# cdcseacave/openMVS

Measured on AMD Instinct MI355X. Metric: Mpix/s depth-map output at 1920x1080 N-view, higher is better.
Workload: dtype f32

## Files before the change

### openmvs_amd/csrc/pm_band.hip

```cpp
#pragma once

#ifndef PM_NDRAW
#define PM_NDRAW 6
#endif
#ifndef PM_BAND_MINWAVES
#define PM_BAND_MINWAVES 3
#endif
#ifndef PM_BAND_MINWAVES_PHOTO
#define PM_BAND_MINWAVES_PHOTO 4
#endif
#ifndef PM_BAND_MINWAVES_PHOTO
#define PM_BAND_MINWAVES_PHOTO 4
#endif

struct PMPix {
	float depth, nx, ny, nz, conf;
	float p0, p1, scaleRange, depthRange;
	int st, it, idxScale, flags;
	float hd, hnx, hny, hnz, hp0, hp1;
	int hst, pad0;
	float nb[2][5];
	float qX[4][3], qn[4][3];
	float vx, vy, normSq0, sumW;
	double X0x, X0y;
	int x, y;
	float x1[2];
	double hr[3];
	float dr[PM_NDRAW][3];
};
#if defined(__HIP_DEVICE_COMPILE__)
#define PM_LDS __attribute__((address_space(3)))
template <class T> __device__ __forceinline__ PM_LDS T* pm_launder(T* p) { PM_LDS T* q = (PM_LDS T*)p; asm volatile("" : "+v"(q)); return q; }
#else
#define PM_LDS
template <class T> __device__ __forceinline__ T* pm_launder(T* p) { return p; }
#endif
enum { PMF_SMOOTH = 1, PMF_CHANGED = 2, PMF_POK0 = 4, PMF_POK1 = 8 };

template <int G, int VPL, bool GEO, bool BUF, bool TILED>
__device__ __forceinline__ void pm_visit(const PMTask& t, const PMKParams& kp, const PMImgBuf& rs, uint32_t pass, int sgn, float2* s_wg, PMPix* s_pixg, const double* hotBase,
		int g, int v, int slot, bool active, int x, int y, int ySafe, size_t idx, const bool* bok, const int* qxs, const int* qys, const size_t* qis, unsigned oldMask,
		float n0D, float n0N0, float n0N1, float n0N2, float n0C, float n1D, float n1N0, float n1N1, float n1N2, float n1C,
		float& rD, float& rN0, float& rN1, float& rN2, float& rC, bool& wr PM_PROF_ARG) {
	constexpr int NBD = PM_SRC_HOT + (GEO ? PM_SRC_GEO : 0);
	const pm_gf gDepth = pm_globw(t.depth), gNormal = pm_globw(t.normal), gConf = pm_globw(t.conf);
	const int yTop = ySafe;
	float oDepth = 0.f, oNx = 0.f, oNy = 0.f, oNz = 0.f, oConf = 2.f, prior = 0.f;
	float myD = 0.f, myN0 = 0.f, myN1 = 0.f, myN2 = 1.f;
	unsigned char maskByte = 1;
	if (active) {
		if (t.prior) prior = pm_glob(t.prior)[idx];
		if (t.mask != nullptr) maskByte = t.mask[idx];
		if (slot == 0) { myD = bok[0] ? n0D : 0.f; myN0 = n0N0; myN1 = n0N1; myN2 = n0N2; }
		else if (slot == 1) { myD = bok[1] ? n1D : 0.f; myN0 = n1N0; myN1 = n1N1; myN2 = n1N2; }
		else {
			const size_t qi = slot == 2 ? qis[2] : qis[3];
			const bool old = TILED && ((oldMask >> slot) & 1u);
			const pm_gcf sD = pm_glob(old ? t.depthOld : t.depth), sN = pm_glob(old ? t.normalOld : t.normal);
			myD = sD[qi]; myN0 = sN[qi * 3]; myN1 = sN[qi * 3 + 1]; myN2 = sN[qi * 3 + 2];
		}
		oDepth = gDepth[idx]; oNx = gNormal[idx * 3]; oNy = gNormal[idx * 3 + 1]; oNz = gNormal[idx * 3 + 2]; oConf = gConf[idx];
	}
	float normSq0, sumW;
	pm_fill_patch<G, true>(t, active, active ? x : PM_HW, active ? y : yTop, v, s_wg, normSq0, sumW);
	const bool masked = active && maskByte == 0;
	const bool valid = active && !masked && !(normSq0 < kp.thMagnitudeSq && !(prior > 0));
	if (v == 0) s_wg[PM_NT] = make_float2(prior, prior > 0 ? pm_expf(normSq0 * (-1.f / (1.f * 0.02f))) : 0.f);
	{
		PM_LDS PMPix* P = pm_launder(s_pixg);
		const bool bk = slot == 0 ? bok[0] : slot == 1 ? bok[1] : slot == 2 ? bok[2] : bok[3];
		const bool okS = valid && bk && myD > 0;
		const unsigned long long bal = __ballot(okS);
		const unsigned closeMask = (unsigned)((bal >> (g * G)) & 0xFull);
		if (v < 4) {
			const int qx = slot == 0 ? qxs[0] : slot == 1 ? qxs[1] : slot == 2 ? qxs[2] : qxs[3];
			const int qy = slot == 0 ? qys[0] : slot == 1 ? qys[1] : slot == 2 ? qys[2] : qys[3];
			const double z = (double)myD;
			P->qX[slot][0] = okS ? (float)(((double)qx - t.cx) * z / t.fx) : 0.f;
			P->qX[slot][1] = okS ? (float)(((double)qy - t.cy) * z / t.fy) : 0.f;
			P->qX[slot][2] = okS ? (float)z : 0.f;
			P->qn[slot][0] = okS ? myN0 : 0.f; P->qn[slot][1] = okS ? myN1 : 0.f; P->qn[slot][2] = okS ? myN2 : 1.f;
		}
		if (v == 0) {
			const double X0x = ((double)x - t.cx) / t.fx, X0y = ((double)y - t.cy) / t.fy;
			P->X0x = X0x; P->X0y = X0y; P->vx = (float)X0x; P->vy = (float)X0y; P->normSq0 = normSq0; P->sumW = sumW; P->x = x; P->y = y;
			P->depth = valid ? oDepth : 0.f; P->nx = valid ? oNx : 0.f; P->ny = valid ? oNy : 0.f; P->nz = valid ? oNz : 0.f; P->conf = valid ? oConf : 2.f;
			P->p0 = 0.f; P->p1 = 0.f; P->scaleRange = 1.f; P->depthRange = 0.f;
			enum { ST_PROP0 = 0, ST_DONE = 5 };
			P->st = valid ? ST_PROP0 : ST_DONE; P->it = 0; P->idxScale = 0;
			P->flags = PMF_SMOOTH | ((closeMask & 1u) ? PMF_POK0 : 0) | ((closeMask & 2u) ? PMF_POK1 : 0) | (int)(closeMask << 8);
			P->nb[0][0] = n0D; P->nb[0][1] = n0N0; P->nb[0][2] = n0N1; P->nb[0][3] = n0N2; P->nb[0][4] = n0C;
			P->nb[1][0] = n1D; P->nb[1][1] = n1N0; P->nb[1][2] = n1N1; P->nb[1][3] = n1N2; P->nb[1][4] = n1C;
		}
		if (v < 2)
			P->x1[v] = v == 0 ? (float)(((double)(x + sgn) - t.cx) / t.fx) : (float)(((double)(y + sgn) - t.cy) / t.fy);
		const unsigned nd = min((unsigned)PM_NDRAW, kp.nRandomIters);
		for (unsigned it0 = 0; it0 < nd; it0 += G) {
			const unsigned itv = it0 + (unsigned)v;
			const PmPhilox4 r = pm_philox4x32_10((uint32_t)x, (uint32_t)y, (uint32_t)(PM_STREAM_REFINE * 256) + itv, 0u, t.k0, t.k1base + pass);
			if (itv < (unsigned)PM_NDRAW) {
				P->dr[itv][0] = 2.f * pm_u32_to_unit(r.v[0]) - 1.f; P->dr[itv][1] = 2.f * pm_u32_to_unit(r.v[1]) - 1.f; P->dr[itv][2] = 2.f * pm_u32_to_unit(r.v[2]) - 1.f;
			}
		}
	}
	__syncthreads();
	PM_TICK(12); PM_COUNT(9, 1);
	enum { ST_PROP0 = 0, ST_PROP1 = 1, ST_DECIDE = 2, ST_RAND = 3, ST_REFINE = 4, ST_DONE = 5 };
	const uint32_t k1 = t.k1base + pass;
	for (;;) {
		bool need = false;
		float hd = 0.f, hnx = 0.f, hny = 0.f, hnz = 1.f;
		{
			PM_LDS PMPix* P = pm_launder(s_pixg);
			int st = P->st; unsigned it = (unsigned)P->it, idxScale = (unsigned)P->idxScale; int flags = P->flags;
			const int px = P->x, py = P->y;
			const float vx = P->vx, vy = P->vy, vz = 1.f;
			float scaleRange = P->scaleRange, depthRange = P->depthRange, p0 = P->p0, p1 = P->p1;
			float hp0 = 0.f, hp1 = 0.f; int hst = ST_DONE;
			while (!need && st != ST_DONE) {
				if (st <= ST_PROP1) {
					const bool vert = (st == ST_PROP1); ++st;
					const bool pok = (flags & (vert ? PMF_POK1 : PMF_POK0)) != 0;
					const PM_LDS float* nbp = P->nb[vert ? 1 : 0];
					const float cd = nbp[0], cnx = nbp[1], cny = nbp[2], cnz = nbp[3], pconf = nbp[4];
					hd = cd; hnx = cnx; hny = cny; hnz = cnz;
					if (pok && pconf < kp.thKeep) {
						float depthNew = cd; bool zero;
						{
							const float nx1 = vert ? vy : vx, cn = vert ? cny : cnx;
							const float denom = cnz + nx1 * cn;
							zero = pm_fabsf(denom) < 0.0001f;
							const float x1 = P->x1[vert ? 1 : 0];
							const float nom = cd * (cnz + x1 * cn);
							if (!zero) depthNew = nom / denom;
						}
						hd = (!zero && pm_in_range(depthNew, t.dMin, t.dMax)) ? depthNew : cd;
						hnx = cnx; hny = cny; hnz = cnz;
						pm_correct_normal(vx, vy, vz, hnx, hny, hnz);
						need = true; hst = ST_PROP0;
					}
				} else if (st == ST_DECIDE) {
					const float conf = P->conf;
					if (conf <= kp.thConfSmall) idxScale = 2;
					else if (conf <= kp.thConfBig) idxScale = 1;
					else if (conf >= kp.thConfRand) { flags &= ~PMF_SMOOTH; st = ST_RAND; it = 0; continue; }
					scaleRange = pm_pow2neg(idxScale);
					depthRange = P->depth * kp.depthRatio;
					p0 = pm_atan2f(P->ny, P->nx); p1 = pm_acosf(pm_clampf(P->nz, -1.f, 1.f));
					st = ST_REFINE; it = 0;
				} else if (st == ST_RAND) {
					if (it >= kp.nRandomIters) { st = ST_DONE; break; }
					const PmPhilox4 r = pm_philox4x32_10((uint32_t)px, (uint32_t)py, (uint32_t)(PM_STREAM_RAND * 256) + it, 0u, t.k0, k1);
					++it;
					const float rr = t.dMinSqr + (t.dMaxSqr - t.dMinSqr) * pm_u32_to_unit(r.v[0]);
					hd = rr * rr;
					pm_random_normal(pm_u32_to_unit(r.v[1]), pm_u32_to_unit(r.v[2]), vx, vy, vz, hnx, hny, hnz);
					need = true; hst = ST_RAND;
				} else {
					if (it >= kp.nRandomIters) { st = ST_DONE; break; }
					float e0, e1, e2;
					if (it < (unsigned)PM_NDRAW) { e0 = P->dr[it][0]; e1 = P->dr[it][1]; e2 = P->dr[it][2]; }
					else {
						const PmPhilox4 r = pm_philox4x32_10((uint32_t)px, (uint32_t)py, (uint32_t)(PM_STREAM_REFINE * 256) + it, 0u, t.k0, k1);
						e0 = 2.f * pm_u32_to_unit(r.v[0]) - 1.f; e1 = 2.f * pm_u32_to_unit(r.v[1]) - 1.f; e2 = 2.f * pm_u32_to_unit(r.v[2]) - 1.f;
					}
					++it;
					const float ndepth = P->depth + (depthRange * scaleRange) * e0;
					if (!pm_in_range(ndepth, t.dMin, t.dMax)) continue;
					hp0 = p0 + (kp.angle1Range * scaleRange) * e1;
					hp1 = p1 + (kp.angle2Range * scaleRange) * e2;
					pm_dir2normal_quad(hp0, hp1, v, hnx, hny, hnz);
					if (hnx * vx + hny * vy + hnz * vz >= 0) continue;
					hd = ndepth;
					need = true; hst = ST_REFINE;
				}
			}
			double hr0 = 0.0, hr1 = 0.0, hr2 = 0.0;
			if (need) pm_homography_plane(P->X0x, P->X0y, hd, hnx, hny, hnz, hr0, hr1, hr2);
			__builtin_amdgcn_wave_barrier();
			if (v == 0) {
				P->hr[0] = hr0; P->hr[1] = hr1; P->hr[2] = hr2;
				P->st = st; P->it = (int)it; P->idxScale = (int)idxScale; P->flags = flags;
				P->scaleRange = scaleRange; P->depthRange = depthRange; P->p0 = p0; P->p1 = p1;
				P->hd = hd; P->hnx = hnx; P->hny = hny; P->hnz = hnz; P->hp0 = hp0; P->hp1 = hp1; P->hst = hst;
			}
		}
		const unsigned long long needBal = __ballot(need);
		if (needBal == 0ull) break;
		PM_TICK(1); PM_COUNT(8, __popcll(needBal)); PM_HIST(__popcll(needBal) / G);
		float sf0, sf1, sf2, sf3;
		{
			const PM_LDS PMPix* P = pm_launder(s_pixg);
			const int flags = P->flags;
			const bool on = need && (flags & PMF_SMOOTH) && ((flags >> (8 + slot)) & 1);
			float myF = 1.f;
			if (on) {
				const float vx = P->vx, vy = P->vy;
				const float q0 = P->qX[slot][0], q1 = P->qX[slot][1], q2 = P->qX[slot][2], m0 = P->qn[slot][0], m1 = P->qn[slot][1], m2 = P->qn[slot][2];
				const float planeD = -hd * (hnx * vx + hny * vy + hnz * 1.f);
				const float dist = (hnx * q0 + (hny * q1 + hnz * q2)) + planeD;
				const float r = dist / hd;
				const float factorDepth = pm_expf((r * r) * kp.smoothSigmaDepth);
				const float ca = pm_clampf((hnx * m0 + hny * m1 + hnz * m2) / pm_sqrtf((hnx * hnx + hny * hny + hnz * hnz) * (m0 * m0 + m1 * m1 + m2 * m2)), -1.f, 1.f);
				const float ac = pm_acosf(ca);
				const float factorNormal = pm_expf((ac * ac) * kp.smoothSigmaNormal);
				myF = (1.f - kp.smoothBonusDepth * factorDepth) * (1.f - kp.smoothBonusNormal * factorNormal);
			}
			sf0 = pm_quad_bcast<0>(myF); sf1 = pm_quad_bcast<1>(myF); sf2 = pm_quad_bcast<2>(myF); sf3 = pm_quad_bcast<3>(myF);
		}
		PM_TICK(2);
		float sc = PM_INF, sc2 = PM_INF;
		{
			const PM_LDS PMPix* P = pm_launder(s_pixg);
#pragma unroll 1
			for (int u = 0; u < VPL; ++u) {
				const int vw = v + u * G;
				if (need && vw < t.nSrc) {
					const float s1 = pm_score_view<GEO, BUF ? 2 : 1, true, true>(t.src[vw], t, kp, P->x, P->y, P->X0x, P->X0y, P->normSq0, P->sumW, s_wg, hd, hnx, hny, hnz, sf0, sf1, sf2, sf3, 0.f,
						hotBase + vw * NBD, hotBase + vw * NBD + PM_SRC_HOT, rs PM_PROF_PASS, (const double*)P->hr);
					if (s1 < sc) { sc2 = sc; sc = s1; } else if (s1 < sc2) sc2 = s1;
				}
			}
		}
		const float nconf = pm_aggregate<G>(sc, t.nSrc, kp.thRobust, sc2);
		{
			PM_LDS PMPix* P = pm_launder(s_pixg);
			if (need && v == 0 && P->conf > nconf) {
				P->conf = nconf; P->depth = P->hd; P->nx = P->hnx; P->ny = P->hny; P->nz = P->hnz;
				int flags = P->flags | PMF_CHANGED;
				P->flags = flags;
				const int hst = P->hst;
				if (hst == ST_RAND) { if (nconf < kp.thConfRand) P->st = ST_DECIDE; }
				else if (hst == ST_REFINE) { P->p0 = P->hp0; P->p1 = P->hp1; const int is = P->idxScale + 1; P->idxScale = is; P->scaleRange = pm_pow2neg((unsigned)is); }
			}
		}
		__builtin_amdgcn_wave_barrier();
		PM_TICK(6);
	}
	{
		const PM_LDS PMPix* P = pm_launder(s_pixg);
		wr = (P->flags & PMF_CHANGED) && valid;
		rD = wr ? P->depth : oDepth; rN0 = wr ? P->nx : oNx; rN1 = wr ? P->ny : oNy; rN2 = wr ? P->nz : oNz; rC = wr ? P->conf : oConf;
	}
}

template <int G, int VPL, bool GEO, bool BUF, bool TILED>
__global__ __launch_bounds__(64, (GEO ? PM_BAND_MINWAVES : PM_BAND_MINWAVES_PHOTO)) void pm_sweep2_kernel(const PMTask* __restrict__ tasks, PMKParams kp, PMStep st, uint32_t pass) {
	constexpr int PPW = 64 / G;
	constexpr int NV = G * VPL;
	constexpr int NBD = PM_SRC_HOT + (GEO ? PM_SRC_GEO : 0);
	static_assert(G >= 4, "a pixel gets at least a quad of lanes");
	PM_PROF_DECL;
	__shared__ float2 s_w[PPW][PM_NT + 1];
	__shared__ double s_src[NV * NBD];
	__shared__ PMPix s_pix[PPW];
	unsigned vbx = blockIdx.x, vby = blockIdx.y;
	{
		const unsigned nbx = gridDim.x, nwg = nbx * gridDim.y, orig = blockIdx.y * nbx + blockIdx.x;
		const unsigned xcd = orig % 8u, q = nwg / 8u, r = nwg % 8u;
		const unsigned wgid = (xcd < r ? xcd * (q + 1u) : r * (q + 1u) + (xcd - r) * q) + orig / 8u;
		vby = wgid / nbx; vbx = wgid - vby * nbx;
	}
	const PMTask& t = tasks[vby];
	const PMImgBuf rs = pm_make_imgbuf(t);
	const int lane = threadIdx.x;
	for (int i = lane; i < NV * NBD; i += 64) s_src[i] = ((const double*)&t.src[i / NBD])[i % NBD];
	const int g = lane / G, v = lane % G, slot = v & 3;
	const int w = t.w, h = t.h;
	const PMStepPix sp = pm_step_pixel<TILED>(st, w, h, (int)vbx * PPW + g);
	const bool active = sp.active;
	const int x = sp.x, y = sp.y;
	const size_t idx = (size_t)y * w + x;
	const int sgn = st.dir == 0 ? -1 : 1;
	bool bok[4]; int qxs[4], qys[4]; size_t qis[4];
#pragma unroll
	for (int k = 0; k < 4; ++k) {
		const int ox = (k == 0) ? sgn : (k == 2 ? -sgn : 0), oy = (k == 1) ? sgn : (k == 3 ? -sgn : 0);
		bool ok;
		if (ox == -1) ok = x > PM_HW; else if (ox == 1) ok = x < w - PM_HW; else if (oy == -1) ok = y > PM_HW; else ok = y < h - PM_HW;
		bok[k] = ok && active; qxs[k] = x + ox; qys[k] = y + oy;
		qis[k] = bok[k] ? (size_t)(y + oy) * w + (x + ox) : idx;
	}
	const pm_gf gDepth = pm_globw(t.depth), gNormal = pm_globw(t.normal), gConf = pm_globw(t.conf);
	float n0D = 0.f, n0N0 = 0.f, n0N1 = 0.f, n0N2 = 0.f, n0C = 2.f, n1D = 0.f, n1N0 = 0.f, n1N1 = 0.f, n1N2 = 0.f, n1C = 2.f;
	if (active) {
		const size_t q0 = qis[0], q1 = qis[1];
		if (TILED) {
			const pm_gcf nD0 = pm_glob((sp.oldMask & 1u) ? t.depthOld : t.depth), nN0 = pm_glob((sp.oldMask & 1u) ? t.normalOld : t.normal), nC0 = pm_glob((sp.oldMask & 1u) ? t.confOld : t.conf);
			const pm_gcf nD1 = pm_glob((sp.oldMask & 2u) ? t.depthOld : t.depth), nN1 = pm_glob((sp.oldMask & 2u) ? t.normalOld : t.normal), nC1 = pm_glob((sp.oldMask & 2u) ? t.confOld : t.conf);
			n0D = nD0[q0]; n0N0 = nN0[q0 * 3]; n0N1 = nN0[q0 * 3 + 1]; n0N2 = nN0[q0 * 3 + 2]; n0C = nC0[q0];
			n1D = nD1[q1]; n1N0 = nN1[q1 * 3]; n1N1 = nN1[q1 * 3 + 1]; n1N2 = nN1[q1 * 3 + 2]; n1C = nC1[q1];
		} else {
			n0D = gDepth[q0]; n0N0 = gNormal[q0 * 3]; n0N1 = gNormal[q0 * 3 + 1]; n0N2 = gNormal[q0 * 3 + 2]; n0C = gConf[q0];
			n1D = gDepth[q1]; n1N0 = gNormal[q1 * 3]; n1N1 = gNormal[q1 * 3 + 1]; n1N2 = gNormal[q1 * 3 + 2]; n1C = gConf[q1];
		}
	}
	__syncthreads();
	float rD, rN0, rN1, rN2, rC; bool wr;
	pm_visit<G, VPL, GEO, BUF, TILED>(t, kp, rs, pass, sgn, s_w[g], &s_pix[g], s_src, g, v, slot, active, x, y, active ? y : PM_HW, active ? idx : (size_t)PM_HW * w + PM_HW, bok, qxs, qys, qis, sp.oldMask,
		n0D, n0N0, n0N1, n0N2, n0C, n1D, n1N0, n1N1, n1N2, n1C, rD, rN0, rN1, rN2, rC, wr PM_PROF_PASS);
	if (wr && v == 0) { gDepth[idx] = rD; gNormal[idx * 3] = rN0; gNormal[idx * 3 + 1] = rN1; gNormal[idx * 3 + 2] = rN2; gConf[idx] = rC; }
	PM_PROF_FLUSH();
}
```

### openmvs_amd/csrc/pm_kernels.hip

```cpp
#pragma once
#include <hip/hip_runtime.h>
#include <cstddef>
#include "pm_math.h"

#define PM_MAX_SRC 16
#ifndef PM_BLOCK
#define PM_BLOCK 64
#endif
typedef const float __attribute__((address_space(1)))* pm_gcf;
typedef float __attribute__((address_space(1)))* pm_gf;
#if defined(__HIP_DEVICE_COMPILE__)
typedef float pm_f4v __attribute__((ext_vector_type(4)));
typedef const pm_f4v __attribute__((address_space(1)))* pm_gcf4;
__device__ __forceinline__ pm_gcf4 pm_glob4(const float4* p) { return (pm_gcf4)p; }
__device__ __forceinline__ pm_f4v pm_loadq(pm_gcf4 base, unsigned off) { return base[off]; }
#else
typedef const float4* pm_gcf4;
__device__ __forceinline__ pm_gcf4 pm_glob4(const float4* p) { return p; }
__device__ __forceinline__ float4 pm_loadq(pm_gcf4 base, unsigned off) { return base[off]; }
#endif
__device__ __forceinline__ pm_gcf pm_glob(const float* p) { return (pm_gcf)p; }
__device__ __forceinline__ pm_gf pm_globw(float* p) { return (pm_gf)p; }
#define PM_HW 4
#define PM_NT 25
// ... 132 lines not shown
#pragma unroll
				for (int k = 0; k < 3; ++k) t += O[i * 3 + k] * O[k * 3 + j];
				Rm[i * 3 + j] = ((i == j ? 1.f : 0.f) + O[i * 3 + j] * s) + t * (1.f - c);
			}
		const float r0 = Rm[0] * nx + Rm[1] * ny + Rm[2] * nz;
		const float r1 = Rm[3] * nx + Rm[4] * ny + Rm[5] * nz;
		const float r2 = Rm[6] * nx + Rm[7] * ny + Rm[8] * nz;
		nx = r0; ny = r1; nz = r2;
	}
}

#define PM_DPP_F(v, ctrl) __int_as_float(__builtin_amdgcn_update_dpp(__float_as_int(v), __float_as_int(v), (ctrl), 0xf, 0xf, false))
template <int G>
__device__ __forceinline__ void pm_group_min2(float s, float s2, float& m1, float& m2) {
	float a = s, b = s2;
#define PM_MIN2_STEP(ctrl) { const float oa = PM_DPP_F(a, ctrl), ob = PM_DPP_F(b, ctrl); \
		const float na = pm_minf(a, oa), nb = pm_minf(pm_maxf(a, oa), pm_minf(b, ob)); a = na; b = nb; }
	if (G >= 2) PM_MIN2_STEP(0xB1)
	if (G >= 4) PM_MIN2_STEP(0x4E)
	if (G >= 8) PM_MIN2_STEP(0x141)
	if (G >= 16) PM_MIN2_STEP(0x140)
#undef PM_MIN2_STEP
	m1 = a; m2 = b;
}
template <int K> __device__ __forceinline__ float pm_quad_bcast(float v) { return PM_DPP_F(v, K * 0x55); }

__device__ __forceinline__ void pm_dir2normal_quad(float p0, float p1, int v, float& nx, float& ny, float& nz) {
	float s, c;
	pm_sincosf((v & 1) ? p1 : p0, &s, &c);
	const float sx = pm_quad_bcast<0>(s), cx = pm_quad_bcast<0>(c), sy = pm_quad_bcast<1>(s), cy = pm_quad_bcast<1>(c);
	nx = cx * sy; ny = sx * sy; nz = cy;
}

__device__ __forceinline__ void pm_homography_plane(double X0x, double X0y, float depth, float nx, float ny, float nz, double& r0, double& r1, double& r2) {
	const double n0 = (double)nx, n1 = (double)ny, n2 = (double)nz;
	const double ndx = (n0 * X0x + n1 * X0y) + n2;
	const double den = ndx * (double)depth;
	const double inv = (den == 0.0) ? 1e+14 : 1.0 / den;
	r0 = n0 * inv; r1 = n1 * inv; r2 = n2 * inv;
}
__device__ __forceinline__ void pm_homography(const double* hlm, const PMTask& t, double X0x, double X0y,
		float depth, float nx, float ny, float nz, float* H, const double* rpre = nullptr) {
	double Hl[9], Hm[3];
#pragma unroll
	for (int i = 0; i < 9; ++i) Hl[i] = hlm[i];
#pragma unroll
	for (int i = 0; i < 3; ++i) Hm[i] = hlm[9 + i];
	double r0, r1, r2;
	if (rpre) { r0 = rpre[0]; r1 = rpre[1]; r2 = rpre[2]; }
	else pm_homography_plane(X0x, X0y, depth, nx, ny, nz, r0, r1, r2);
#pragma unroll
	for (int i = 0; i < 3; ++i) {
		const double hm = Hm[i];
		const double m0 = Hl[i * 3 + 0] + hm * r0;
		const double m1 = Hl[i * 3 + 1] + hm * r1;
		const double m2 = Hl[i * 3 + 2] + hm * r2;
		if (t.hrUpper) {
			H[i * 3 + 0] = (float)(m0 * t.Hr[0]);
			H[i * 3 + 1] = (float)(m1 * t.Hr[4]);
			H[i * 3 + 2] = (float)((m0 * t.Hr[2] + m1 * t.Hr[5]) + m2 * t.Hr[8]);
		} else {
#pragma unroll
			for (int j = 0; j < 3; ++j)
				H[i * 3 + j] = (float)((m0 * t.Hr[j] + m1 * t.Hr[3 + j]) + m2 * t.Hr[6 + j]);
		}
	}
}

#ifndef PM_WIDE_MINWAVES
#define PM_WIDE_MINWAVES 3
#endif

#if defined(__HIP_DEVICE_COMPILE__)
typedef int pm_rsrc __attribute__((ext_vector_type(4)));
__device__ __forceinline__ pm_rsrc pm_make_rsrc(const void* base, unsigned count, unsigned stride = 16) {
	const unsigned long long b = (unsigned long long)base;
	pm_rsrc r;
	r.x = __builtin_amdgcn_readfirstlane((int)(unsigned)b);
	r.y = __builtin_amdgcn_readfirstlane((int)(((unsigned)(b >> 32) & 0xffffu) | (stride << 16)));
	r.z = __builtin_amdgcn_readfirstlane((int)count);
	r.w = 0x00020000;
	return r;
}
__device__ __forceinline__ void pm_bufload5(pm_f4v& q0, pm_f4v& q1, pm_f4v& q2, pm_f4v& q3, pm_f4v& q4, unsigned i0, unsigned i1, unsigned i2, unsigned i3, unsigned i4, pm_rsrc r) {
	asm volatile("buffer_load_dwordx4 %0, %5, %10, 0 idxen\n\tbuffer_load_dwordx4 %1, %6, %10, 0 idxen\n\tbuffer_load_dwordx4 %2, %7, %10, 0 idxen\n\t"
	             "buffer_load_dwordx4 %3, %8, %10, 0 idxen\n\tbuffer_load_dwordx4 %4, %9, %10, 0 idxen"
		: "=&v"(q0), "=&v"(q1), "=&v"(q2), "=&v"(q3), "=&v"(q4) : "v"(i0), "v"(i1), "v"(i2), "v"(i3), "v"(i4), "s"(r) : "memory");
}
template <int LEFT>
__device__ __forceinline__ void pm_bufwait5(pm_f4v& q0, pm_f4v& q1, pm_f4v& q2, pm_f4v& q3, pm_f4v& q4) {
	asm volatile("s_waitcnt vmcnt(%5)" : "+v"(q0), "+v"(q1), "+v"(q2), "+v"(q3), "+v"(q4) : "i"(LEFT));
}
__device__ __forceinline__ unsigned pm_mad24(int a, int b, unsigned c) { unsigned r; asm("v_mad_u32_u24 %0, %1, %2, %3" : "=v"(r) : "v"(a), "v"(b), "v"(c)); return r; }
#else
typedef float4 pm_f4v;
struct pm_rsrc { const float4* base; unsigned count; };
__device__ __forceinline__ pm_rsrc pm_make_rsrc(const void* base, unsigned count) { return pm_rsrc{(const float4*)base, count}; }
__device__ __forceinline__ void pm_bufload5(pm_f4v& q0, pm_f4v& q1, pm_f4v& q2, pm_f4v& q3, pm_f4v& q4, unsigned i0, unsigned i1, unsigned i2, unsigned i3, unsigned i4, pm_rsrc r) {
	const float4 z = make_float4(0.f, 0.f, 0.f, 0.f);
	q0 = i0 < r.count ? r.base[i0] : z; q1 = i1 < r.count ? r.base[i1] : z; q2 = i2 < r.count ? r.base[i2] : z; q3 = i3 < r.count ? r.base[i3] : z; q4 = i4 < r.count ? r.base[i4] : z;
}
template <int LEFT> __device__ __forceinline__ void pm_bufwait5(pm_f4v&, pm_f4v&, pm_f4v&, pm_f4v&, pm_f4v&) {}
__device__ __forceinline__ unsigned pm_mad24(int a, int b, unsigned c) { return (unsigned)(((unsigned)a & 0xffffffu) * ((unsigned)b & 0xffffffu)) + c; }
#endif

struct PMImgBuf { pm_rsrc rs; };
__device__ __forceinline__ PMImgBuf pm_make_imgbuf(const PMTask& t) {
	PMImgBuf b;
	b.rs = pm_make_rsrc(t.qArr, t.qCount);
	return b;
}

template <bool QUAD>
__device__ __forceinline__ void pm_tap_row_global(const pm_gcf img, int sw, int sh, float h0, float h3, float h6, float X0, float X1, float X2,
		const float2* wrow, float& sum, float& sumSq, float& num, bool& oob)
{
	const int lxMax = sw - 2, lyMax = sh - 2;
	float fxs[5], fys[5];
	unsigned offs[5];
#pragma unroll
	for (int j = 0; j < 5; ++j) {
		float ptx, pty;
		pm_div2(X0, X1, X2, &ptx, &pty);
		oob = oob || !pm_inside1(ptx, pty, sw, sh);
		int lx = (int)ptx, ly = (int)pty;
		fxs[j] = ptx - (float)lx; fys[j] = pty - (float)ly;
		lx = min(max(lx, 0), lxMax); ly = min(max(ly, 0), lyMax);
		offs[j] = QUAD ? 4u * ((unsigned)(lx + ly) * (unsigned)sh + (unsigned)ly) : (unsigned)ly * (unsigned)sw + (unsigned)lx;
		X0 += h0; X1 += h3; X2 += h6;
	}
	float v00[5], v01[5], v10[5], v11[5];
#pragma unroll
	for (int j = 0; j < 5; ++j) {
		const pm_gcf p = img + offs[j];
		if (QUAD) { v00[j] = p[0]; v01[j] = p[1]; v10[j] = p[2]; v11[j] = p[3]; }
		else { v00[j] = p[0]; v01[j] = p[1]; v10[j] = p[sw]; v11[j] = p[sw + 1]; }
	}
#pragma unroll
// ... 51 lines not shown
		sumSq += v * vw;
		num += v * pw.y;
	}
}
template <bool BUF>
__device__ __forceinline__ void pm_taps_fast(const PMImgBuf& rs, unsigned qbase, const pm_gcf4 imgQ, int sw, int sh, const float* H, float bX0, float bX1, float bX2,
		const float2* wts, float& sum, float& sumSq, float& num, PMTapRange& rg)
{
	PMRowPos pa, pb; PMRowQ qa, qb;
	pm_row_issue<BUF, true>(rs, qbase, imgQ, sw, sh, H[0], H[3], H[6], bX0, bX1, bX2, pa, qa, rg);
#pragma unroll 1
	for (int i = 0; i < 4; i += 2) {
		bX0 += H[1]; bX1 += H[4]; bX2 += H[7];
		pm_row_issue<BUF, false>(rs, qbase, imgQ, sw, sh, H[0], H[3], H[6], bX0, bX1, bX2, pb, qb, rg);
		PM_SCHED_BARRIER();
		pm_row_consume<BUF, 5>(pa, qa, wts + i * 5, sum, sumSq, num);
		PM_SCHED_BARRIER();
		bX0 += H[1]; bX1 += H[4]; bX2 += H[7];
		pm_row_issue<BUF, false>(rs, qbase, imgQ, sw, sh, H[0], H[3], H[6], bX0, bX1, bX2, pa, qa, rg);
		PM_SCHED_BARRIER();
		pm_row_consume<BUF, 5>(pb, qb, wts + (i + 1) * 5, sum, sumSq, num);
		PM_SCHED_BARRIER();
	}
	pm_range_corner(rg, pa.ptx[0], pa.pty[0], bX2);
	pm_range_corner(rg, pa.ptx[4], pa.pty[4], (((bX2 + H[6]) + H[6]) + H[6]) + H[6]);
	pm_row_consume<BUF, 0>(pa, qa, wts + 20, sum, sumSq, num);
}

template <bool GEO, int MODE, bool PF = false, bool EARLY = false>
__device__ __forceinline__ float pm_score_view(const PMSrcView& s, const PMTask& t, const PMKParams& kp,
		int x, int y, double X0x, double X0y, float normSq0, float sumW, const float2* wts,
		float depth, float nx, float ny, float nz,
		float sf0, float sf1, float sf2, float sf3, float prior,
		const double* hot, const double* geoTab, const PMImgBuf& rs PM_PROF_ARG, const double* rpre = nullptr)
{
	const int sw = ((const int*)(hot + 12))[0], sh = ((const int*)(hot + 12))[1];
	float H[9];
	pm_homography(hot, t, X0x, X0y, depth, nx, ny, nz, H, rpre);
	PM_TICK(3);
	const float px = (float)(x - PM_HW), py = (float)(y - PM_HW);
	const float X0 = H[0] * px + H[1] * py + H[2];
	const float X1 = H[3] * px + H[4] * py + H[5];
	const float X2 = H[6] * px + H[7] * py + H[8];
	float bX0 = X0, bX1 = X1, bX2 = X2;
#pragma unroll
	for (int i = 0; i < 9; ++i) H[i] *= 2.f;
	float sum = 0.f, sumSq = 0.f, num = 0.f;
	bool oob = false;
	if (MODE == 0) {
#pragma unroll 1
		for (int i = 0; i < 5; ++i) {
			pm_tap_row_global<false>(pm_glob(s.img), sw, sh, H[0], H[3], H[6], bX0, bX1, bX2, wts + i * 5, sum, sumSq, num, oob);
			bX0 += H[1]; bX1 += H[4]; bX2 += H[7];
		}
	} else {
		const bool sane = pm_fabsf(X0) + 8.f * (pm_fabsf(H[0]) + pm_fabsf(H[1])) < 5e17f && pm_fabsf(X1) + 8.f * (pm_fabsf(H[3]) + pm_fabsf(H[4])) < 5e17f
			&& pm_fabsf(X2) + 8.f * (pm_fabsf(H[6]) + pm_fabsf(H[7])) < 5e11f;
		if (EARLY && sane) {
			bool outside = false;
			float cx, cy;
			if (bX2 >= 9.094947e-13f && bX2 <= 1.0995116e12f) { pm_div2_inrange(bX0, bX1, bX2, &cx, &cy); outside = !pm_inside1(cx, cy, sw, sh); }
			float c0 = bX0, c1 = bX1, c2 = bX2;
#pragma unroll
			for (int i = 0; i < 4; ++i) { c0 += H[1]; c1 += H[4]; c2 += H[7]; }
#pragma unroll
			for (int j = 0; j < 4; ++j) { c0 += H[0]; c1 += H[3]; c2 += H[6]; }
			if (c2 >= 9.094947e-13f && c2 <= 1.0995116e12f) { pm_div2_inrange(c0, c1, c2, &cx, &cy); outside = outside || !pm_inside1(cx, cy, sw, sh); }
// ... 17 lines not shown
			oob = !cornersIn;
			if (cornersIn && !allIn) {
				float cX0 = rX0, cX1 = rX1, cX2 = rX2;
#pragma unroll 1
				for (int i = 0; i < 5; ++i) {
					float X0t = cX0, X1t = cX1, X2t = cX2;
#pragma unroll 1
					for (int j = 0; j < 5; ++j) {
						float ptx, pty;
						pm_div2_inrange(X0t, X1t, X2t, &ptx, &pty);
						oob = oob || !pm_inside1(ptx, pty, sw, sh);
						X0t += H[0]; X1t += H[3]; X2t += H[6];
					}
					cX0 += H[1]; cX1 += H[4]; cX2 += H[7];
				}
			}
		} else {
			sum = 0.f; sumSq = 0.f; num = 0.f;
			bX0 = rX0; bX1 = rX1; bX2 = rX2;
#pragma unroll 1
			for (int i = 0; i < 5; ++i) {
				pm_tap_row_global<true>(pm_glob((const float*)s.imgQ), sw, sh, H[0], H[3], H[6], bX0, bX1, bX2, wts + i * 5, sum, sumSq, num, oob);
				bX0 += H[1]; bX1 += H[4]; bX2 += H[7];
			}
		}
	}
	PM_TICK(4);
	if (oob) return kp.thRobust;
	const float normSq1 = sumSq - (sum * sum) / sumW;
	const float nrmSq = normSq0 * normSq1;
	if (nrmSq <= 1e-16f) return kp.thRobust;
	const float ncc = pm_clampf(num / pm_sqrtf(nrmSq), -1.f, 1.f);
	float score = 1.f - ncc;
	score *= sf0; score *= sf1; score *= sf2; score *= sf3;
	if (GEO) {
		const float* gt = (const float*)geoTab;
		const float* sdepth = *(const float* const*)(geoTab + 12);
		const int dw = ((const int*)(geoTab + 13))[0], dh = ((const int*)(geoTab + 13))[1];
		float Tl[9], Tm[3], Tr[9], Tn[3];
#pragma unroll
		for (int i = 0; i < 9; ++i) { Tl[i] = gt[i]; Tr[i] = gt[12 + i]; }
#pragma unroll
		for (int i = 0; i < 3; ++i) { Tm[i] = gt[9 + i]; Tn[i] = gt[21 + i]; }
#pragma unroll
		for (int i = 0; i < 9; ++i) PM_OPAQUE(Tr[i]);
#pragma unroll
		for (int i = 0; i < 3; ++i) PM_OPAQUE(Tn[i]);
		if (sdepth != nullptr) {
			float consistency = 4.f;
			const float Xc0 = (float)X0x * depth, Xc1 = (float)X0y * depth, Xc2 = depth;
			const float Y0 = (Tl[0] * Xc0 + Tl[1] * Xc1 + Tl[2] * Xc2) + Tm[0];
			const float Y1 = (Tl[3] * Xc0 + Tl[4] * Xc1 + Tl[5] * Xc2) + Tm[1];
			const float Y2 = (Tl[6] * Xc0 + Tl[7] * Xc1 + Tl[8] * Xc2) + Tm[2];
			if (Y2 > 0) {
				const float x1x = Y0 / Y2, x1y = Y1 / Y2;
				if (pm_inside1(x1x, x1y, dw, dh)) {
					const int lx = (int)x1x, ly = (int)x1y;
					const float fx = x1x - (float)lx, fx1 = 1.f - fx;
					const float fy = x1y - (float)ly, fy1 = 1.f - fy;
					const pm_gcf p = pm_glob(sdepth) + (size_t)ly * dw + lx;
					const float x0y0 = p[0], x1y0 = p[1], x0y1 = p[dw], x1y1 = p[dw + 1];
					const bool b00 = pm_fabsf(Y2 - x0y0) / Y2 < 0.03f, b10 = pm_fabsf(Y2 - x1y0) / Y2 < 0.03f;
					const bool b01 = pm_fabsf(Y2 - x0y1) / Y2 < 0.03f, b11 = pm_fabsf(Y2 - x1y1) / Y2 < 0.03f;
					if (b00 || b10 || b01 || b11) {
						const float depth1 =
							fy1 * (fx1 * (b00 ? x0y0 : (b10 ? x1y0 : (b01 ? x0y1 : x1y1))) + fx * (b10 ? x1y0 : (b00 ? x0y0 : (b11 ? x1y1 : x0y1)))) +
// ... 494 lines not shown
```

Baseline: 55.85.

## Switch band kernel lane mapping from pixel-major to view-major groups

Lanes are remapped so that consecutive lanes hold different pixels for the same view slot (g = lane % PPW, v = lane / PPW). Neighbouring pixels' texture gathers for one view then sit in the same quads, and per-pixel loads are restricted to the lanes that need them. Reductions and the normal construction move from quad DPP broadcasts to cross-lane xor shuffles at stride PPW, and smoothness factors go through LDS (nb is reused as scratch) instead of quad broadcasts. A host-side gather census instrumentation is added behind a compile flag. The risks are costlier cross-lane shuffles and extra LDS traffic with wave barriers.

```diff
diff --git a/openmvs_amd/csrc/pm_band.hip b/openmvs_amd/csrc/pm_band.hip
--- a/openmvs_amd/csrc/pm_band.hip
+++ b/openmvs_amd/csrc/pm_band.hip
@@ -13,13 +13,13 @@
 #define PM_BAND_MINWAVES_PHOTO 4
 #endif
 
-struct PMPix {
+struct alignas(16) PMPix {
+	float nb[2][5];
 	float depth, nx, ny, nz, conf;
 	float p0, p1, scaleRange, depthRange;
 	int st, it, idxScale, flags;
 	float hd, hnx, hny, hnz, hp0, hp1;
 	int hst, pad0;
-	float nb[2][5];
 	float qX[4][3], qn[4][3];
 	float vx, vy, normSq0, sumW;
 	double X0x, X0y;
@@ -35,43 +35,49 @@
 #define PM_LDS
 template <class T> __device__ __forceinline__ T* pm_launder(T* p) { return p; }
 #endif
+static_assert(sizeof(PMPix) == 368, "sixteen of them, the weights and the views' matrices fit a sixteenth of a CU's LDS (tests/test_kernel_resources.py)");
+__device__ __forceinline__ PM_LDS float* pm_pix_sf(PM_LDS PMPix* P) { return P->nb[0]; }
 enum { PMF_SMOOTH = 1, PMF_CHANGED = 2, PMF_POK0 = 4, PMF_POK1 = 8 };
 
 template <int G, int VPL, bool GEO, bool BUF, bool TILED>
 __device__ __forceinline__ void pm_visit(const PMTask& t, const PMKParams& kp, const PMImgBuf& rs, uint32_t pass, int sgn, float2* s_wg, PMPix* s_pixg, const double* hotBase,
-		int g, int v, int slot, bool active, int x, int y, int ySafe, size_t idx, const bool* bok, const int* qxs, const int* qys, const size_t* qis, unsigned oldMask,
+		int g, int v, bool active, int x, int y, int ySafe, size_t idx, const bool* bok, const int* qxs, const int* qys, const size_t* qis, unsigned oldMask,
 		float n0D, float n0N0, float n0N1, float n0N2, float n0C, float n1D, float n1N0, float n1N1, float n1N2, float n1C,
 		float& rD, float& rN0, float& rN1, float& rN2, float& rC, bool& wr PM_PROF_ARG) {
 	constexpr int NBD = PM_SRC_HOT + (GEO ? PM_SRC_GEO : 0);
+	constexpr int PPW = 64 / G;
+	const int slot = v & 3;
 	const pm_gf gDepth = pm_globw(t.depth), gNormal = pm_globw(t.normal), gConf = pm_globw(t.conf);
 	const int yTop = ySafe;
 	float oDepth = 0.f, oNx = 0.f, oNy = 0.f, oNz = 0.f, oConf = 2.f, prior = 0.f;
 	float myD = 0.f, myN0 = 0.f, myN1 = 0.f, myN2 = 1.f;
 	unsigned char maskByte = 1;
-	if (active) {
-		if (t.prior) prior = pm_glob(t.prior)[idx];
-		if (t.mask != nullptr) maskByte = t.mask[idx];
-		if (slot == 0) { myD = bok[0] ? n0D : 0.f; myN0 = n0N0; myN1 = n0N1; myN2 = n0N2; }
-		else if (slot == 1) { myD = bok[1] ? n1D : 0.f; myN0 = n1N0; myN1 = n1N1; myN2 = n1N2; }
+	if (active && v < 4) {
+		if (v == 0) {
+			if (t.prior) prior = pm_glob(t.prior)[idx];
+			if (t.mask != nullptr) maskByte = t.mask[idx];
+			oDepth = gDepth[idx]; oNx = gNormal[idx * 3]; oNy = gNormal[idx * 3 + 1]; oNz = gNormal[idx * 3 + 2]; oConf = gConf[idx];
+			myD = bok[0] ? n0D : 0.f; myN0 = n0N0; myN1 = n0N1; myN2 = n0N2;
+		}
+		else if (v == 1) { myD = bok[1] ? n1D : 0.f; myN0 = n1N0; myN1 = n1N1; myN2 = n1N2; }
 		else {
 			const size_t qi = slot == 2 ? qis[2] : qis[3];
 			const bool old = TILED && ((oldMask >> slot) & 1u);
 			const pm_gcf sD = pm_glob(old ? t.depthOld : t.depth), sN = pm_glob(old ? t.normalOld : t.normal);
 			myD = sD[qi]; myN0 = sN[qi * 3]; myN1 = sN[qi * 3 + 1]; myN2 = sN[qi * 3 + 2];
 		}
-		oDepth = gDepth[idx]; oNx = gNormal[idx * 3]; oNy = gNormal[idx * 3 + 1]; oNz = gNormal[idx * 3 + 2]; oConf = gConf[idx];
 	}
 	float normSq0, sumW;
 	pm_fill_patch<G, true>(t, active, active ? x : PM_HW, active ? y : yTop, v, s_wg, normSq0, sumW);
-	const bool masked = active && maskByte == 0;
-	const bool valid = active && !masked && !(normSq0 < kp.thMagnitudeSq && !(prior > 0));
+	const bool valid0 = v == 0 && active && maskByte != 0 && !(normSq0 < kp.thMagnitudeSq && !(prior > 0));
+	const bool valid = ((__ballot(valid0) >> g) & 1ull) != 0;
 	if (v == 0) s_wg[PM_NT] = make_float2(prior, prior > 0 ? pm_expf(normSq0 * (-1.f / (1.f * 0.02f))) : 0.f);
 	{
 		PM_LDS PMPix* P = pm_launder(s_pixg);
 		const bool bk = slot == 0 ? bok[0] : slot == 1 ? bok[1] : slot == 2 ? bok[2] : bok[3];
 		const bool okS = valid && bk && myD > 0;
-		const unsigned long long bal = __ballot(okS);
-		const unsigned closeMask = (unsigned)((bal >> (g * G)) & 0xFull);
+		const unsigned long long bal = __ballot(okS) >> g;
+		const unsigned closeMask = (unsigned)((bal & 1ull) | ((bal >> (PPW - 1)) & 2ull) | ((bal >> (2 * PPW - 2)) & 4ull) | ((bal >> (3 * PPW - 3)) & 8ull));
 		if (v < 4) {
 			const int qx = slot == 0 ? qxs[0] : slot == 1 ? qxs[1] : slot == 2 ? qxs[2] : qxs[3];
 			const int qy = slot == 0 ? qys[0] : slot == 1 ? qys[1] : slot == 2 ? qys[2] : qys[3];
@@ -89,11 +95,11 @@
 			enum { ST_PROP0 = 0, ST_DONE = 5 };
 			P->st = valid ? ST_PROP0 : ST_DONE; P->it = 0; P->idxScale = 0;
 			P->flags = PMF_SMOOTH | ((closeMask & 1u) ? PMF_POK0 : 0) | ((closeMask & 2u) ? PMF_POK1 : 0) | (int)(closeMask << 8);
-			P->nb[0][0] = n0D; P->nb[0][1] = n0N0; P->nb[0][2] = n0N1; P->nb[0][3] = n0N2; P->nb[0][4] = n0C;
-			P->nb[1][0] = n1D; P->nb[1][1] = n1N0; P->nb[1][2] = n1N1; P->nb[1][3] = n1N2; P->nb[1][4] = n1C;
-		}
-		if (v < 2)
+		}
+		if (v < 2) {
+			P->nb[v][0] = v == 0 ? n0D : n1D; P->nb[v][1] = v == 0 ? n0N0 : n1N0; P->nb[v][2] = v == 0 ? n0N1 : n1N1; P->nb[v][3] = v == 0 ? n0N2 : n1N2; P->nb[v][4] = v == 0 ? n0C : n1C;
 			P->x1[v] = v == 0 ? (float)(((double)(x + sgn) - t.cx) / t.fx) : (float)(((double)(y + sgn) - t.cy) / t.fy);
+		}
 		const unsigned nd = min((unsigned)PM_NDRAW, kp.nRandomIters);
 		for (unsigned it0 = 0; it0 < nd; it0 += G) {
 			const unsigned itv = it0 + (unsigned)v;
@@ -108,6 +114,7 @@
 	enum { ST_PROP0 = 0, ST_PROP1 = 1, ST_DECIDE = 2, ST_RAND = 3, ST_REFINE = 4, ST_DONE = 5 };
 	const uint32_t k1 = t.k1base + pass;
 	for (;;) {
+		PM_CENSUS_TRIP();
 		bool need = false;
 		float hd = 0.f, hnx = 0.f, hny = 0.f, hnz = 1.f;
 		{
@@ -169,7 +176,7 @@
 					if (!pm_in_range(ndepth, t.dMin, t.dMax)) continue;
 					hp0 = p0 + (kp.angle1Range * scaleRange) * e1;
 					hp1 = p1 + (kp.angle2Range * scaleRange) * e2;
-					pm_dir2normal_quad(hp0, hp1, v, hnx, hny, hnz);
+					pm_dir2normal_vm<PPW>(hp0, hp1, v, hnx, hny, hnz);
 					if (hnx * vx + hny * vy + hnz * vz >= 0) continue;
 					hd = ndepth;
 					need = true; hst = ST_REFINE;
@@ -188,11 +195,10 @@
 		const unsigned long long needBal = __ballot(need);
 		if (needBal == 0ull) break;
 		PM_TICK(1); PM_COUNT(8, __popcll(needBal)); PM_HIST(__popcll(needBal) / G);
-		float sf0, sf1, sf2, sf3;
 		{
-			const PM_LDS PMPix* P = pm_launder(s_pixg);
+			PM_LDS PMPix* P = pm_launder(s_pixg);
 			const int flags = P->flags;
-			const bool on = need && (flags & PMF_SMOOTH) && ((flags >> (8 + slot)) & 1);
+			const bool on = need && v < 4 && (flags & PMF_SMOOTH) && ((flags >> (8 + slot)) & 1);
 			float myF = 1.f;
 			if (on) {
 				const float vx = P->vx, vy = P->vy;
@@ -206,7 +212,8 @@
 				const float factorNormal = pm_expf((ac * ac) * kp.smoothSigmaNormal);
 				myF = (1.f - kp.smoothBonusDepth * factorDepth) * (1.f - kp.smoothBonusNormal * factorNormal);
 			}
-			sf0 = pm_quad_bcast<0>(myF); sf1 = pm_quad_bcast<1>(myF); sf2 = pm_quad_bcast<2>(myF); sf3 = pm_quad_bcast<3>(myF);
+			if (v < 4) pm_pix_sf(P)[slot] = myF;
+			__builtin_amdgcn_wave_barrier();
 		}
 		PM_TICK(2);
 		float sc = PM_INF, sc2 = PM_INF;
@@ -216,13 +223,15 @@
 			for (int u = 0; u < VPL; ++u) {
 				const int vw = v + u * G;
 				if (need && vw < t.nSrc) {
-					const float s1 = pm_score_view<GEO, BUF ? 2 : 1, true, true>(t.src[vw], t, kp, P->x, P->y, P->X0x, P->X0y, P->normSq0, P->sumW, s_wg, hd, hnx, hny, hnz, sf0, sf1, sf2, sf3, 0.f,
-						hotBase + vw * NBD, hotBase + vw * NBD + PM_SRC_HOT, rs PM_PROF_PASS, (const double*)P->hr);
+					PM_CENSUS_VIEW(t.w, G, u);
+					const float s1 = pm_score_view<GEO, BUF ? 2 : 1, true, true>(t.src[vw], t, kp, P->x, P->y, P->X0x, P->X0y, P->normSq0, P->sumW, s_wg, hd, hnx, hny, hnz, 1.f, 1.f, 1.f, 1.f, 0.f,
+						hotBase + vw * NBD, hotBase + vw * NBD + PM_SRC_HOT, rs PM_PROF_PASS, (const double*)P->hr, (const float*)pm_pix_sf((PM_LDS PMPix*)P));
+					PM_CENSUS_VIEW_END();
 					if (s1 < sc) { sc2 = sc; sc = s1; } else if (s1 < sc2) sc2 = s1;
 				}
 			}
 		}
-		const float nconf = pm_aggregate<G>(sc, t.nSrc, kp.thRobust, sc2);
+		const float nconf = pm_aggregate_vm<G>(sc, t.nSrc, kp.thRobust, sc2);
 		{
 			PM_LDS PMPix* P = pm_launder(s_pixg);
 			if (need && v == 0 && P->conf > nconf) {
@@ -265,7 +274,7 @@
 	const PMImgBuf rs = pm_make_imgbuf(t);
 	const int lane = threadIdx.x;
 	for (int i = lane; i < NV * NBD; i += 64) s_src[i] = ((const double*)&t.src[i / NBD])[i % NBD];
-	const int g = lane / G, v = lane % G, slot = v & 3;
+	const int g = lane % PPW, v = lane / PPW;
 	const int w = t.w, h = t.h;
 	const PMStepPix sp = pm_step_pixel<TILED>(st, w, h, (int)vbx * PPW + g);
 	const bool active = sp.active;
@@ -283,21 +292,21 @@
 	}
 	const pm_gf gDepth = pm_globw(t.depth), gNormal = pm_globw(t.normal), gConf = pm_globw(t.conf);
 	float n0D = 0.f, n0N0 = 0.f, n0N1 = 0.f, n0N2 = 0.f, n0C = 2.f, n1D = 0.f, n1N0 = 0.f, n1N1 = 0.f, n1N2 = 0.f, n1C = 2.f;
-	if (active) {
+	if (active && v < 2) {
 		const size_t q0 = qis[0], q1 = qis[1];
 		if (TILED) {
 			const pm_gcf nD0 = pm_glob((sp.oldMask & 1u) ? t.depthOld : t.depth), nN0 = pm_glob((sp.oldMask & 1u) ? t.normalOld : t.normal), nC0 = pm_glob((sp.oldMask & 1u) ? t.confOld : t.conf);
 			const pm_gcf nD1 = pm_glob((sp.oldMask & 2u) ? t.depthOld : t.depth), nN1 = pm_glob((sp.oldMask & 2u) ? t.normalOld : t.normal), nC1 = pm_glob((sp.oldMask & 2u) ? t.confOld : t.conf);
-			n0D = nD0[q0]; n0N0 = nN0[q0 * 3]; n0N1 = nN0[q0 * 3 + 1]; n0N2 = nN0[q0 * 3 + 2]; n0C = nC0[q0];
-			n1D = nD1[q1]; n1N0 = nN1[q1 * 3]; n1N1 = nN1[q1 * 3 + 1]; n1N2 = nN1[q1 * 3 + 2]; n1C = nC1[q1];
+			if (v == 0) { n0D = nD0[q0]; n0N0 = nN0[q0 * 3]; n0N1 = nN0[q0 * 3 + 1]; n0N2 = nN0[q0 * 3 + 2]; n0C = nC0[q0]; }
+			else { n1D = nD1[q1]; n1N0 = nN1[q1 * 3]; n1N1 = nN1[q1 * 3 + 1]; n1N2 = nN1[q1 * 3 + 2]; n1C = nC1[q1]; }
 		} else {
-			n0D = gDepth[q0]; n0N0 = gNormal[q0 * 3]; n0N1 = gNormal[q0 * 3 + 1]; n0N2 = gNormal[q0 * 3 + 2]; n0C = gConf[q0];
-			n1D = gDepth[q1]; n1N0 = gNormal[q1 * 3]; n1N1 = gNormal[q1 * 3 + 1]; n1N2 = gNormal[q1 * 3 + 2]; n1C = gConf[q1];
+			if (v == 0) { n0D = gDepth[q0]; n0N0 = gNormal[q0 * 3]; n0N1 = gNormal[q0 * 3 + 1]; n0N2 = gNormal[q0 * 3 + 2]; n0C = gConf[q0]; }
+			else { n1D = gDepth[q1]; n1N0 = gNormal[q1 * 3]; n1N1 = gNormal[q1 * 3 + 1]; n1N2 = gNormal[q1 * 3 + 2]; n1C = gConf[q1]; }
 		}
 	}
 	__syncthreads();
 	float rD, rN0, rN1, rN2, rC; bool wr;
-	pm_visit<G, VPL, GEO, BUF, TILED>(t, kp, rs, pass, sgn, s_w[g], &s_pix[g], s_src, g, v, slot, active, x, y, active ? y : PM_HW, active ? idx : (size_t)PM_HW * w + PM_HW, bok, qxs, qys, qis, sp.oldMask,
+	pm_visit<G, VPL, GEO, BUF, TILED>(t, kp, rs, pass, sgn, s_w[g], &s_pix[g], s_src, g, v, active, x, y, active ? y : PM_HW, active ? idx : (size_t)PM_HW * w + PM_HW, bok, qxs, qys, qis, sp.oldMask,
 		n0D, n0N0, n0N1, n0N2, n0C, n1D, n1N0, n1N1, n1N2, n1C, rD, rN0, rN1, rN2, rC, wr PM_PROF_PASS);
 	if (wr && v == 0) { gDepth[idx] = rD; gNormal[idx * 3] = rN0; gNormal[idx * 3 + 1] = rN1; gNormal[idx * 3 + 2] = rN2; gConf[idx] = rC; }
 	PM_PROF_FLUSH();
diff --git a/openmvs_amd/csrc/pm_kernels.hip b/openmvs_amd/csrc/pm_kernels.hip
--- a/openmvs_amd/csrc/pm_kernels.hip
+++ b/openmvs_amd/csrc/pm_kernels.hip
@@ -188,6 +188,39 @@
 	nx = cx * sy; ny = sx * sy; nz = cy;
 }
 
+template <int PPW> __device__ __forceinline__ float pm_lane_xor(float v, int o = PPW) {
+	if (PPW == 8 && o == 8) return PM_DPP_F(v, 0x128);
+	return __shfl_xor(v, o, 64);
+}
+template <int G>
+__device__ __forceinline__ void pm_group_min2_vm(float s, float s2, float& m1, float& m2) {
+	constexpr int PPW = 64 / G;
+	float a = s, b = s2;
+#pragma unroll
+	for (int o = PPW; o < 64; o <<= 1) {
+		const float oa = pm_lane_xor<PPW>(a, o), ob = pm_lane_xor<PPW>(b, o);
+		const float na = pm_minf(a, oa), nb = pm_minf(pm_maxf(a, oa), pm_minf(b, ob)); a = na; b = nb;
+	}
+	m1 = a; m2 = b;
+}
+template <int G>
+__device__ __forceinline__ float pm_aggregate_vm(float viewScore, int nSrc, float thRobust, float viewScore2) {
+	float m1, m2;
+	pm_group_min2_vm<G>(viewScore, viewScore2, m1, m2);
+	if (nSrc <= 1) return m1;
+	if (m2 >= thRobust) return m1;
+	return (m1 + m2) / 2.f;
+}
+template <int PPW>
+__device__ __forceinline__ void pm_dir2normal_vm(float p0, float p1, int v, float& nx, float& ny, float& nz) {
+	const bool odd = (v & 1) != 0;
+	float s, c;
+	pm_sincosf(odd ? p1 : p0, &s, &c);
+	const float os = pm_lane_xor<PPW>(s), oc = pm_lane_xor<PPW>(c);
+	const float sx = odd ? os : s, cx = odd ? oc : c, sy = odd ? s : os, cy = odd ? c : oc;
+	nx = cx * sy; ny = sx * sy; nz = cy;
+}
+
 __device__ __forceinline__ void pm_homography_plane(double X0x, double X0y, float depth, float nx, float ny, float nz, double& r0, double& r1, double& r2) {
 	const double n0 = (double)nx, n1 = (double)ny, n2 = (double)nz;
 	const double ndx = (n0 * X0x + n1 * X0y) + n2;
@@ -252,7 +285,71 @@
 typedef float4 pm_f4v;
 struct pm_rsrc { const float4* base; unsigned count; };
 __device__ __forceinline__ pm_rsrc pm_make_rsrc(const void* base, unsigned count) { return pm_rsrc{(const float4*)base, count}; }
+#if defined(PM_GATHER_CENSUS)
+#include <algorithm>
+#include <array>
+namespace pm_census {
+struct Rec { unsigned key; unsigned lane; unsigned idx[5]; };
+struct Stat { unsigned long long loads = 0, lanes = 0, blocksVM = 0, blocksPM = 0, quadsVM[5] = {0, 0, 0, 0, 0}; };
+inline std::vector<Rec> recs;
+inline std::map<int, Stat> stats;
+inline unsigned long long wgLaunch = ~0ull; inline unsigned wgX = 0, wgY = 0; inline int wgWidth = 0, wgG = 4;
+inline unsigned trips[64], curKey = 0, curRow = 0; inline bool armed = false;
+inline unsigned blocksOfQuads(const std::array<unsigned, 64>& blk, unsigned long long on, unsigned long long* hist) {
+	unsigned total = 0;
+	for (int q = 0; q < 16; ++q) {
+		unsigned seen[4]; int n = 0;
+		for (int l = 4 * q; l < 4 * q + 4; ++l) if ((on >> l) & 1ull) { bool dup = false; for (int k = 0; k < n; ++k) dup = dup || seen[k] == blk[l]; if (!dup) seen[n++] = blk[l]; }
+		total += (unsigned)n; if (hist) hist[n]++;
+	}
+	return total;
+}
+inline void flush() {
+	if (recs.empty()) return;
+	std::stable_sort(recs.begin(), recs.end(), [](const Rec& a, const Rec& b) { return a.key < b.key; });
+	Stat& s = stats[wgWidth];
+	const int G = wgG, PPW = 64 / G;
+	for (size_t i = 0; i < recs.size();) {
+		size_t j = i; while (j < recs.size() && recs[j].key == recs[i].key) ++j;
+		for (int k = 0; k < 5; ++k) {
+			std::array<unsigned, 64> vm{}, pm{}; unsigned long long onVM = 0, onPM = 0;
+			for (size_t r = i; r < j; ++r) {
+				const unsigned l = recs[r].lane, g = l % PPW, v = l / PPW, lp = g * G + v;
+				vm[l] = recs[r].idx[k] >> 2; onVM |= 1ull << l; pm[lp] = recs[r].idx[k] >> 2; onPM |= 1ull << lp;
+			}
+			s.loads++; s.lanes += (unsigned long long)(j - i);
+			s.blocksVM += blocksOfQuads(vm, onVM, s.quadsVM); s.blocksPM += blocksOfQuads(pm, onPM, nullptr);
+		}
+		i = j;
+	}
+	recs.clear();
+}
+inline void report() {
+	flush();
+	for (auto& kv : stats) {
+		const Stat& s = kv.second; const double L = (double)s.loads, Q = 16.0 * L;
+		fprintf(stderr, "gather census: level width %d: %llu tap wave-loads, %.1f active lanes per load; blocks per load: view-major (shipped) %.2f, pixel-major %.2f, ratio %.3f; "
+			"blocks per quad (shipped) %.3f; quads touching 0/1/2/3/4 blocks: %.1f %.1f %.1f %.1f %.1f %%\n", kv.first, s.loads, s.lanes / L, s.blocksVM / L, s.blocksPM / L,
+			(double)s.blocksVM / (double)s.blocksPM, s.blocksVM / Q, 100.0 * s.quadsVM[0] / Q, 100.0 * s.quadsVM[1] / Q, 100.0 * s.quadsVM[2] / Q, 100.0 * s.quadsVM[3] / Q, 100.0 * s.quadsVM[4] / Q);
+	}
+}
+inline void enter() {
+	static bool reg = false; if (!reg) { reg = true; atexit(report); }
+	if (wgLaunch != hipemu::launches || wgX != blockIdx.x || wgY != blockIdx.y) { flush(); wgLaunch = hipemu::launches; wgX = blockIdx.x; wgY = blockIdx.y; for (unsigned& t : trips) t = 0; }
+}
+inline void trip() { enter(); trips[threadIdx.x & 63]++; }
+inline void view(int width, int G, int u) { wgWidth = width; wgG = G; curKey = (trips[threadIdx.x & 63] * 8u + (unsigned)u) * 8u; curRow = 0; armed = true; }
+inline void viewEnd() { armed = false; }
+inline void note(unsigned i0, unsigned i1, unsigned i2, unsigned i3, unsigned i4) { if (armed) recs.push_back(Rec{curKey + curRow++, threadIdx.x & 63u, {i0, i1, i2, i3, i4}}); }
+}
+#define PM_CENSUS_TRIP() pm_census::trip()
+#define PM_CENSUS_VIEW(width, G, u) pm_census::view((width), (G), (u))
+#define PM_CENSUS_VIEW_END() pm_census::viewEnd()
+#endif
 __device__ __forceinline__ void pm_bufload5(pm_f4v& q0, pm_f4v& q1, pm_f4v& q2, pm_f4v& q3, pm_f4v& q4, unsigned i0, unsigned i1, unsigned i2, unsigned i3, unsigned i4, pm_rsrc r) {
+#if defined(PM_GATHER_CENSUS)
+	pm_census::note(i0, i1, i2, i3, i4);
+#endif
 	const float4 z = make_float4(0.f, 0.f, 0.f, 0.f);
 	q0 = i0 < r.count ? r.base[i0] : z; q1 = i1 < r.count ? r.base[i1] : z; q2 = i2 < r.count ? r.base[i2] : z; q3 = i3 < r.count ? r.base[i3] : z; q4 = i4 < r.count ? r.base[i4] : z;
 }
@@ -260,6 +357,11 @@
 __device__ __forceinline__ unsigned pm_mad24(int a, int b, unsigned c) { return (unsigned)(((unsigned)a & 0xffffffu) * ((unsigned)b & 0xffffffu)) + c; }
 #endif
 
+#ifndef PM_CENSUS_TRIP
+#define PM_CENSUS_TRIP()
+#define PM_CENSUS_VIEW(width, G, u)
+#define PM_CENSUS_VIEW_END()
+#endif
 struct PMImgBuf { pm_rsrc rs; };
 __device__ __forceinline__ PMImgBuf pm_make_imgbuf(const PMTask& t) {
 	PMImgBuf b;
@@ -377,7 +479,7 @@
 		int x, int y, double X0x, double X0y, float normSq0, float sumW, const float2* wts,
 		float depth, float nx, float ny, float nz,
 		float sf0, float sf1, float sf2, float sf3, float prior,
-		const double* hot, const double* geoTab, const PMImgBuf& rs PM_PROF_ARG, const double* rpre = nullptr)
+		const double* hot, const double* geoTab, const PMImgBuf& rs PM_PROF_ARG, const double* rpre = nullptr, const float* sfp = nullptr)
 {
 	const int sw = ((const int*)(hot + 12))[0], sh = ((const int*)(hot + 12))[1];
 	float H[9];
@@ -461,6 +563,7 @@
 	if (nrmSq <= 1e-16f) return kp.thRobust;
 	const float ncc = pm_clampf(num / pm_sqrtf(nrmSq), -1.f, 1.f);
 	float score = 1.f - ncc;
+	if (sfp) { sf0 = sfp[0]; sf1 = sfp[1]; sf2 = sfp[2]; sf3 = sfp[3]; }
 	score *= sf0; score *= sf1; score *= sf2; score *= sf3;
 	if (GEO) {
 		const float* gt = (const float*)geoTab;
```

New measurement: 57.33 (median of 6 runs). +2.6%, better.
